# kurtkuehnert/bevy_terrain

Hardware: AMD Instinct MI355X
Metric: terrain tiles/sec preprocessed (16k^2 heightmap) (higher is better)
Workload: dtype f32; 1 GPU; synthetic 16384x16384 fBm R16 heightmap (seed 42), T=512, b=2, lod_count=6: split + pyramid + stitch into 1365 tiles; jobs_in_flight=1, ranks_seen=1, all_gather_bytes_per_rank=0

## Files before the change

### bevy_terrain_amd/csrc/bt_fused.hip

```cpp
#include <cstdio>
#include <cstdlib>
#include <type_traits>

#include "bt_internal.hpp"

namespace bt {

namespace {

constexpr uint32_t kInvalid = 0xFFFFFFFFu;

#include "bt_stitch.hpp"

#ifdef BT_DEBUG_HOOKS
#define BT_ABLATE(A, bits) ((A).ablate & (bits))
#else
#define BT_ABLATE(A, bits) 0u
#endif
constexpr uint32_t kMainRows = 8;
#ifndef BT_DMA_POS
#define BT_DMA_POS 0
#endif

constexpr uint32_t kDmaPos = BT_DMA_POS;
constexpr uint32_t kMaxBorder = 8;

struct MainItem {
    uint32_t side, x, y, atlas_index, raster;
};

struct FusedArgs {
    AttachmentMeta m;
    uint16_t* atlas;
    const RasterDev* rasters;
    const MainItem* items;
    const uint32_t* grids;
    uint32_t grid_lod_lo, grid_lod_hi, grid_sides;
    uint32_t regular, reg_first;
    const TaskDev* seam_tasks;
    uint32_t seam_count, seam_skip;
    uint32_t seam_pull;
    uint32_t tail_extras;
    float tlx, tly, brx, bry;
    uint32_t lod;
    uint32_t levels;
    uint32_t item_count;
    uint32_t groups;
    uint32_t sides;
    uint32_t lds_pitch;
    uint32_t lds_rows;
    uint32_t apron_lods;
    uint32_t rotate_priority;
    uint32_t apron_cols;
    uint32_t prev_zero;
    uint32_t apron_global;
    uint32_t single_buffer;
    uint32_t ablate;
};

__device__ __forceinline__ float unorm16_to_float(uint32_t t) {
    const float x = float(t);
    const float r = 1.0f / 65535.0f;
    const float q0 = x * r;
    const float e = __builtin_fmaf(-q0, 65535.0f, x);
    return __builtin_fmaf(e, r, q0);
}
__device__ __forceinline__ uint32_t float_to_unorm16(float e) {
    const float cl = __builtin_amdgcn_fmed3f(e, 0.0f, 1.0f);
    return uint32_t(0.5f + 65535.0f * cl);
}
__device__ __forceinline__ float mixf(float a, float b, float t) { return a * (1.0f - t) + b * t; }

struct Axis {
    int i0, i1;
    float fr;
};

__host__ __device__ __forceinline__ Axis split_axis(uint32_t r, uint32_t c, uint32_t tile, float scale, float lo, float hi, uint32_t dim) {
    const float tc = float(r) / float(c);
// ... 179 lines not shown
            out |= uint32_t(0.5f + (255.0f / 256.0f) * (sum * 0.25f)) << sh;
        }
        return out;
    }
    float value[4] = {0.0f, 0.0f, 0.0f, 0.0f}, count = 0.0f;
#pragma unroll
    for (int i = 0; i < 4; i++)
        if ((t[i] & 0x00FFFFFFu) != 0) {
#pragma unroll
            for (int k = 0; k < 4; k++) value[k] += unorm8_to_float((t[i] >> (8 * k)) & 0xFFu);
            count += 1.0f;
        }
    if (count == 0.0f) return 0;
    uint32_t out = 0;
#pragma unroll
    for (int k = 0; k < 4; k++) {
        const float e = value[k] / count;
        const float cl = e < 0.0f ? 0.0f : (e > 1.0f ? 1.0f : e);
        out |= uint32_t(floorf(0.5f + 255.0f * cl)) << (8 * k);
    }
    return out;
}

__device__ __forceinline__ uint32_t split_value_slow(const FusedArgs& A, const RasterDev& r, uint32_t tx, uint32_t rx, uint32_t ty,
                                                  uint32_t ry, uint32_t home_index) {
    const float scale = float(1u << A.lod);
    const uint32_t c = A.m.center_size, b = A.m.border_size, T = A.m.texture_size;
    const Axis ax = split_axis(rx, c, tx, scale, A.tlx, A.brx, r.width);
    const Axis ay = split_axis(ry, c, ty, scale, A.tly, A.bry, r.height);
    typedef const uint8_t __attribute__((address_space(1))) * global_bytes;
    typedef const uint16_t __attribute__((address_space(1))) * global_u16;
    const global_u16 row0 = (global_u16)((global_bytes)r.data + uint64_t(ay.i0) * r.pitch);
    const global_u16 row1 = (global_u16)((global_bytes)r.data + uint64_t(ay.i1) * r.pitch);
    const uint32_t t00 = row0[ax.i0], t10 = row0[ax.i1], t01 = row1[ax.i0], t11 = row1[ax.i1];
    if (t00 == 0 || t10 == 0 || t01 == 0 || t11 == 0) {
        if (home_index == kInvalid || A.prev_zero) return 0;
        return A.atlas[uint64_t(home_index) * T * T + uint64_t(b + ry) * T + b + rx];
    }
    const float top = mixf(unorm16_to_float(t00), unorm16_to_float(t10), ax.fr);
    const float bot = mixf(unorm16_to_float(t01), unorm16_to_float(t11), ax.fr);
    return float_to_unorm16(mixf(top, bot, ay.fr));
}

__device__ __forceinline__ uint32_t xcd_remap(uint32_t bid, uint32_t total) {
    const uint32_t q = total / 8u, r = total % 8u, xcd = bid % 8u, i = bid / 8u;
    return (xcd < r ? xcd * (q + 1u) : r * (q + 1u) + (xcd - r) * q) + i;
}

__device__ __forceinline__ int wave_min(int v) {
#pragma unroll
    for (int o = 32; o > 0; o >>= 1) v = min(v, __shfl_xor(v, o));
    return v;
// ... 1 lines not shown
__device__ __forceinline__ int wave_max(int v) {
#pragma unroll
    for (int o = 32; o > 0; o >>= 1) v = max(v, __shfl_xor(v, o));
    return v;
}

struct RowParam {
    int y0, y1;
    float fy;
    uint32_t pad;
};

constexpr uint32_t kMaxChunks = 64;
struct MainShared {
    int row_y0[kMaxChunks * kMainRows];
    float2 row_fy[kMaxChunks * kMainRows];
    int win_ymin[kMaxChunks];
    uint32_t win_slots[kMaxChunks];
    RowParam apron[2 * kMaxBorder];
    int xmin, xmax;
    uint32_t pad_[2];
};
static_assert(sizeof(MainShared) % 16 == 0, "LDS carve must stay 16-byte aligned");

struct Texel4 {
    float a0, a1, b0, b1;
    uint32_t za, zb;
};

__device__ __forceinline__ Texel4 convert4(uint32_t ta0, uint32_t ta1, uint32_t tb0, uint32_t tb1) {
    Texel4 r;
    r.a0 = unorm16_to_float(ta0);
    r.a1 = unorm16_to_float(ta1);
    r.b0 = unorm16_to_float(tb0);
    r.b1 = unorm16_to_float(tb1);
    r.za = min(ta0, ta1);
    r.zb = min(tb0, tb1);
    return r;
}

__device__ __forceinline__ void corner_pixels(const FusedArgs& A, uint32_t item_index, uint32_t tid, uint32_t threads) {
    const MainItem it = A.items[item_index];
    const RasterDev raster = A.rasters[it.raster];
    const uint32_t T = A.m.texture_size, b = A.m.border_size, c = A.m.center_size, o = b + c;
    const uint32_t self = grid_lookup(A, it.side, A.lod, int(it.x), int(it.y));
    for (uint32_t t = tid; t < 4 * b * b; t += threads) {
        const uint32_t corner = t / (b * b), i = (t % (b * b)) % b, j = (t % (b * b)) / b;
        const bool left = corner == 0 || corner == 3, top = corner < 2;
        const uint32_t px = left ? i : o + i, py = top ? j : o + j;
        const uint32_t n = grid_lookup(A, it.side, A.lod, int(it.x) + (left ? -1 : 1), int(it.y) + (top ? -1 : 1));
        uint32_t v;
        if (n != kInvalid)
            v = split_value_slow(A, raster, left ? it.x - 1 : it.x + 1, left ? c - b + i : i, top ? it.y - 1 : it.y + 1, top ? c - b + j : j, n);
        else
            v = split_value_slow(A, raster, it.x, left ? 0u : c - 1, it.y, top ? 0u : c - 1, self);
        A.atlas[uint64_t(self) * T * T + py * T + px] = uint16_t(v);
    }
}

template <bool kStaged, bool kGeneric, uint32_t kT, uint32_t kP, bool kDma = false>
__device__ __forceinline__ void fused_main_chunks(const FusedArgs& A, uint32_t item_index, uint32_t k_begin, uint32_t k_end, uint8_t* smem) {
    MainShared& S = *reinterpret_cast<MainShared*>(smem);
    uint16_t* s_buf = reinterpret_cast<uint16_t*>(smem + sizeof(MainShared));
    constexpr bool kFix = kStaged && !kGeneric;
    const bool one_buffer = kDma && kP == 0 && A.single_buffer != 0;
    const uint32_t buf_texels = one_buffer ? 0u : A.lds_rows * (kP ? kP : A.lds_pitch);

    const MainItem it = A.items[item_index];
    const RasterDev raster = A.rasters[it.raster];
    const uint32_t T = kT ? kT : A.m.texture_size, b = A.m.border_size, c = A.m.center_size, o = b + c;
    const uint32_t tid = threadIdx.x;
#ifdef BT_DEBUG_HOOKS
    auto wg_stamp = [&](uint32_t slot) {
        if (BT_ABLATE(A, 134217728u) && tid == 0 && blockIdx.x < 4096u)
            reinterpret_cast<unsigned long long*>(A.atlas + uint64_t(A.m.atlas_size - 1u) * T * T)[16384u + blockIdx.x * 4u + slot] = __builtin_amdgcn_s_memrealtime();
    };
#else
    auto wg_stamp = [&](uint32_t) {};
#endif
    wg_stamp(0);
    const float scale = float(1u << A.lod);
    const uint32_t tile_texels = T * T;
    const uint32_t chunks_per_tile = (c + kMainRows - 1) / kMainRows;

    const TileNb t5 = load_tile_nb(A, it.side, A.lod, it.x, it.y);
    const uint32_t self4 = A.levels >= 2 ? grid_lookup(A, it.side, A.lod - 1, int(it.x >> 1), int(it.y >> 1)) : kInvalid;
    const uint32_t self3 = A.levels >= 3 ? grid_lookup(A, it.side, A.lod - 2, int(it.x >> 2), int(it.y >> 2)) : kInvalid;

    for (uint32_t i = tid; i < (k_end - k_begin) * kMainRows; i += 256u) {
        const uint32_t cr = k_begin * kMainRows + i;
        if (cr < c) {
            const Axis ay = split_axis(cr, c, it.y, scale, A.tly, A.bry, raster.height);
            S.row_y0[i] = ay.i0 | (ay.i1 == ay.i0 ? int(0x80000000u) : 0);
            S.row_fy[i] = float2{ay.fr, 1.0f - ay.fr};
        }
    }
    if (tid >= 32 && tid < 32 + 2 * b) {
        const uint32_t r = tid - 32, k = r % b;
        const bool top = r < b;
        const uint32_t nrow = top ? t5.n : t5.s;
        uint32_t ty, ry;
        if (nrow != kInvalid) { ty = top ? it.y - 1 : it.y + 1; ry = top ? c - b + k : k; } else { ty = it.y; ry = top ? 0u : c - 1; }
        const Axis ay = split_axis(ry, c, ty, scale, A.tly, A.bry, raster.height);
        S.apron[r].y0 = ay.i0;
        S.apron[r].y1 = ay.i1;
        S.apron[r].fy = ay.fr;
        S.apron[r].pad = ry;
    }

    const uint32_t half_c = c / 2, half_b = b / 2;
    const bool is_centre = tid < half_c;
    const bool is_right = !is_centre && tid < half_c + half_b;
    const bool is_left = !is_centre && !is_right && tid < half_c + 2 * half_b;
    const bool is_idle = !is_centre && !is_right && !is_left;
    uint32_t px0 = 0;
    uint32_t txa = it.x, txb = it.x, rxa = 0, rxb = 0;
    if (is_centre) {
        px0 = b + 2 * tid;
        rxa = 2 * tid;
        rxb = 2 * tid + 1;
    } else if (is_right) {
        const uint32_t j = 2 * (tid - half_c);
        px0 = o + j;
        if (t5.e != kInvalid) { txa = txb = it.x + 1; rxa = j; rxb = j + 1; } else { rxa = rxb = c - 1; }
    } else if (is_left) {
        const uint32_t j = 2 * (tid - half_c - half_b);
        px0 = j;
        if (t5.w != kInvalid) { txa = txb = it.x - 1; rxa = c - b + j; rxb = c - b + j + 1; } else { rxa = rxb = 0; }
    }
    const Axis axa = split_axis(rxa, c, txa, scale, A.tlx, A.brx, raster.width);
    const Axis axb = split_axis(rxb, c, txb, scale, A.tlx, A.brx, raster.width);
    const float fxa = axa.fr, fxb = axb.fr, gxa = 1.0f - fxa, gxb = 1.0f - fxb;
    const uint32_t home_col = is_right && t5.e != kInvalid ? t5.e : (is_left && t5.w != kInvalid ? t5.w : t5.self);

    if (tid == half_c + half_b) S.xmin = min(axa.i0, axb.i0);
    if (tid == half_c + half_b - 1) S.xmax = max(axa.i1, axb.i1);
    __syncthreads();
    if (tid < k_end - k_begin) {
        const uint32_t k = k_begin + tid, n = min(kMainRows, c - k * kMainRows);
        const int* y0 = S.row_y0 + tid * kMainRows;
        const int first = y0[0] & 0x7fffffff;
        bool consecutive = n == kMainRows;
        for (uint32_t i = 0; i < n; i++) consecutive = consecutive && y0[i] == first + int(i);
        int lo = first, hi = (y0[n - 1] & 0x7fffffff) + (y0[n - 1] < 0 ? 0 : 1);
        if (!(kDma && kP == 0 && A.apron_global)) {
            if (k == 0) lo = min(lo, S.apron[0].y0);
            if (k == chunks_per_tile - 1) hi = max(hi, S.apron[2 * b - 1].y1);
        }
        S.win_ymin[tid] = lo;
        S.win_slots[tid] = uint32_t(hi - lo + 1) | (consecutive ? 0x80000000u : 0u);
    }
    __syncthreads();

    const int xa = __builtin_amdgcn_readfirstlane(S.xmin) & ~7;
    const uint32_t P = kP ? kP : A.lds_pitch;
    typedef const uint8_t __attribute__((address_space(1))) * global_bytes;
    typedef const uint16_t __attribute__((address_space(1))) * global_u16;
    typedef uint32_t u32x4 __attribute__((ext_vector_type(4)));
    typedef const u32x4 __attribute__((address_space(1))) * global_u4;
    typedef uint16_t u16x2 __attribute__((ext_vector_type(2)));
    const global_bytes data = (global_bytes)raster.data;
    const uint32_t chunks_per_row = P / 8u;
    const uint32_t row_texels = uint32_t(raster.pitch / 2u);
    const bool wide = ((reinterpret_cast<uintptr_t>(raster.data) | raster.pitch) & 15u) == 0;
    constexpr uint32_t kBatch = 4;

    auto chunk_rows = [&](uint32_t k) -> uint32_t { return min(kMainRows, c - k * kMainRows); };
    auto window = [&](uint32_t k, int& ymin, uint32_t& slots) {
        ymin = __builtin_amdgcn_readfirstlane(S.win_ymin[k - k_begin]);
        slots = uint32_t(__builtin_amdgcn_readfirstlane(S.win_slots[k - k_begin])) & 0x7fffffffu;
    };
    uint32_t src_off[kBatch], lds_off[kBatch];
#pragma unroll
    for (uint32_t i = 0; i < kBatch; i++) {
        const uint32_t ch = tid + 256u * i;
        const uint32_t slot = ch / chunks_per_row, kk = ch - slot * chunks_per_row;
        const uint32_t x = min(uint32_t(xa) + 8u * kk, row_texels - 8u);
        src_off[i] = slot * uint32_t(raster.pitch) + x * 2u;
        lds_off[i] = (slot * P + 8u * kk) * 2u;
    }
    const uint32_t safe_off = src_off[0] - (tid / chunks_per_row) * uint32_t(raster.pitch);
    auto stage_issue = [&](int ymin, uint32_t slots, u32x4 (&v)[kBatch]) {
        const global_bytes base = data + uint64_t(uint32_t(ymin)) * raster.pitch;
        const uint32_t bound = slots * P * 2u;
#pragma unroll
        for (uint32_t i = 0; i < kBatch; i++) {
            const global_u4 ptr = (global_u4)(base + (lds_off[i] < bound ? src_off[i] : safe_off));
            v[i] = BT_ABLATE(A, 32768u) ? __builtin_nontemporal_load(ptr) : *ptr;
        }
    };
    auto stage_commit = [&](uint16_t* s_src, uint32_t slots, const u32x4 (&v)[kBatch]) {
        const uint32_t bound = slots * P * 2u;
        uint8_t* s_bytes = reinterpret_cast<uint8_t*>(s_src);
#pragma unroll
        for (uint32_t i = 0; i < kBatch; i++)
            if (lds_off[i] < bound) *reinterpret_cast<u32x4*>(s_bytes + lds_off[i]) = v[i];
    };
    auto stage_narrow = [&](uint16_t* s_src, int ymin, uint32_t slots) {
        for (uint32_t i = tid; i < slots * P; i += 256u) {
            const uint32_t slot = i / P, kk = i - slot * P;
            const uint32_t x = uint32_t(xa) + kk;
            const global_u16 row = (global_u16)(data + uint64_t(ymin + int(slot)) * raster.pitch);
            s_src[i] = x < raster.width ? row[x] : uint16_t(1);
        }
    };

    typedef __attribute__((address_space(3))) uint8_t* lds_bytes;
    const uint32_t dma_lane = tid & 63u;
    const uint32_t dma_off_main = min(uint32_t(xa) * 2u + dma_lane * 16u, uint32_t(raster.pitch) - 16u);
    const uint32_t dma_off_tail = min(uint32_t(xa) * 2u + 1024u + (dma_lane & 1u) * 16u, uint32_t(raster.pitch) - 16u);
    auto dma_issue = [&](uint16_t* s_dst, int ymin, uint32_t slots) {
        static_assert(!kDma || kP == 528 || kP == 0, "the DMA variants: 1056-byte LDS rows, or a run-time pitch");
        const lds_bytes dst = (lds_bytes)reinterpret_cast<uint8_t*>(s_dst);
        for (uint32_t slot = uint32_t(__builtin_amdgcn_readfirstlane(int(tid >> 6))); slot < slots; slot += 4u) {
            const global_bytes row = data + uint64_t(uint32_t(ymin) + slot) * raster.pitch;
            if constexpr (kP == 528) {
                if (BT_ABLATE(A, 32768u))
                    __builtin_amdgcn_global_load_lds((const __attribute__((address_space(1))) void*)(row + dma_off_main),
                                                     (__attribute__((address_space(3))) void*)(dst + slot * (kP * 2u)), 16, 0, 2);
                else
                __builtin_amdgcn_global_load_lds((const __attribute__((address_space(1))) void*)(row + dma_off_main),
                                                 (__attribute__((address_space(3))) void*)(dst + slot * (kP * 2u)), 16, 0, 0);
                if (dma_lane < 2u)
                    __builtin_amdgcn_global_load_lds((const __attribute__((address_space(1))) void*)(row + dma_off_tail),
                                                     (__attribute__((address_space(3))) void*)(dst + slot * (kP * 2u) + 1024u), 16, 0, 0);
            } else {
                const uint32_t row_bytes = P * 2u;
                for (uint32_t piece = 0; piece < row_bytes; piece += 1024u)
                    if (piece + dma_lane * 16u < row_bytes)
                        __builtin_amdgcn_global_load_lds((const __attribute__((address_space(1))) void*)(row + min(uint32_t(xa) * 2u + piece + dma_lane * 16u, uint32_t(raster.pitch) - 16u)),
                                                         (__attribute__((address_space(3))) void*)(dst + slot * row_bytes + piece), 16, 0, 0);
            }
        }
    };

    uint16_t* tile5 = A.atlas + uint64_t(t5.self) * tile_texels;
    uint32_t* tile5_u32 = reinterpret_cast<uint32_t*>(tile5);
    uint16_t* tile4 = A.atlas + uint64_t(self4 == kInvalid ? 0u : self4) * tile_texels;
    uint16_t* tile3 = A.atlas + uint64_t(self3 == kInvalid ? 0u : self3) * tile_texels;
    const uint32_t cx4 = (it.x & 1u) * half_c + tid, cy4_base = (it.y & 1u) * half_c;
    const uint32_t cx3 = (it.x & 3u) * (c / 4) + (tid >> 1), cy3_base = (it.y & 3u) * (c / 4);
    const bool do4 = A.levels >= 2 && !BT_ABLATE(A, 1u), do3 = A.levels >= 3 && !BT_ABLATE(A, 1u);
    auto make_xpush = [&](uint32_t shift, uint32_t self, uint32_t cx, uint32_t& layer, uint32_t& off, uint32_t& count) {
        layer = 0;
        off = 0;
        count = 0;
        if (!is_centre || self == kInvalid) return;
        const bool left = cx < b, right = cx >= c - b;
        if (!left && !right) return;
        const uint32_t n = grid_lookup(A, it.side, A.lod - shift, int(it.x >> shift) + (left ? -1 : 1), int(it.y >> shift));
        const uint32_t j = left ? cx : cx - (c - b);
        if (n != kInvalid) {
            layer = n;
            off = b * T + (left ? o + j : j);
            count = 1;
        } else if (left ? cx == 0 : cx == c - 1) {
            layer = self;
            off = b * T + (left ? 0u : o);
            count = b;
        }
    };
    uint32_t x4_layer, x4_off, x4_count, x3_layer, x3_off, x3_count;
    make_xpush(1, A.levels >= 2 ? self4 : kInvalid, cx4, x4_layer, x4_off, x4_count);
    make_xpush(2, A.levels >= 3 ? self3 : kInvalid, cx3, x3_layer, x3_off, x3_count);
    auto xpush4 = [&](uint32_t cy, uint16_t v) {
        for (uint32_t e = 0; e < x4_count; e++) A.atlas[uint64_t(x4_layer) * tile_texels + x4_off + cy * T + e] = v;
    };
    auto xpush3 = [&](uint32_t cy, uint16_t v) {
        for (uint32_t e = 0; e < x3_count; e++) A.atlas[uint64_t(x3_layer) * tile_texels + x3_off + cy * T + e] = v;
    };
    const uint32_t la0 = uint32_t(axa.i0 - xa), la1 = uint32_t(axa.i1 - xa), lb0 = uint32_t(axb.i0 - xa), lb1 = uint32_t(axb.i1 - xa);

    int ymin = 0;
    uint32_t slots = 0;
    u32x4 pre[kBatch];
    window(k_begin, ymin, slots);
    if constexpr (kDma) {
        dma_issue(s_buf + (k_begin & 1u) * buf_texels, ymin, slots);
    } else if (kStaged && !BT_ABLATE(A, 8u)) {
        if (wide) {
            stage_issue(ymin, slots, pre);
            stage_commit(s_buf + (k_begin & 1u) * buf_texels, slots, pre);
        } else {
            stage_narrow(s_buf + (k_begin & 1u) * buf_texels, ymin, slots);
        }
    }
    if constexpr (kStaged) {
        if (k_begin == 0) corner_pixels(A, item_index, tid, 256u);
    }
    auto chunk_barrier = [&]() {
        if constexpr (kDma) asm volatile("s_waitcnt vmcnt(0)" ::: "memory");
        __syncthreads();
    };
    uint16_t* s_src = s_buf;
    int cur_ymin = 0;
    auto fetch_row = [&](int y) -> Texel4 {
        if constexpr (kStaged) {
            const uint16_t* row = s_src + uint32_t(y - cur_ymin) * P;
            return convert4(row[la0], row[la1], row[lb0], row[lb1]);
        } else {
            const global_u16 row = (global_u16)(data + uint64_t(y) * raster.pitch);
            return convert4(row[axa.i0], row[axa.i1], row[axb.i0], row[axb.i1]);
        }
    };
    auto apron_rows = [&](uint32_t k, auto gtag) {
        constexpr bool kKeep = decltype(gtag)::value;
        if (!((k == 0 || k == chunks_per_tile - 1) && is_centre)) return;
        for (uint32_t r = 0; r < 2 * b; r++) {
            const bool top = r < b;
            if (top ? k != 0 : k != chunks_per_tile - 1) continue;
            const uint32_t kk = r % b, py = top ? kk : o + kk;
            const int y0 = __builtin_amdgcn_readfirstlane(S.apron[r].y0), y1 = __builtin_amdgcn_readfirstlane(S.apron[r].y1);
// ... 371 lines not shown
                            xpush4(cy4, uint16_t(q0));
                            xpush4(cy4 + 1, uint16_t(q1));
                        }
                        if (do3) {
                            const uint32_t other0 = __shfl_xor(q0, 1), other1 = __shfl_xor(q1, 1);
                            if (is_centre && (tid & 1u) == 0) {
                                const f2 mine = conv2(q0, q1), theirs = conv2(other0, other1);
                                const float s3 = ((mine.x + mine.y) + theirs.x) + theirs.y;
                                uint32_t w3 = uint32_t(0.5f + (0.25f * (65535.0f / 65536.0f)) * s3);
                                if (kFix && min(min(q0, q1), min(other0, other1)) == 0) w3 = downsample4(q0, q1, other0, other1);
                                const uint32_t cy3 = cy3_base + (cy >> 2);
                                tile3[(b + cy3) * T + b + cx3] = uint16_t(w3);
                                if (x3_count) xpush3(cy3, uint16_t(w3));
                            }
                        }
                    }
                }
                }
            } else {
                generic_rows(k);
            }
        }

        if (!more) break;
        if (kStaged && !kDma && !BT_ABLATE(A, 8u)) {
            uint16_t* s_next = s_buf + ((k + 1) & 1u) * buf_texels;
            if (wide) stage_commit(s_next, next_slots, pre);
            else stage_narrow(s_next, next_ymin, next_slots);
        }
        ymin = next_ymin;
        slots = next_slots;
        if constexpr (kDma && kP == 0) {
            if (one_buffer) {
                __syncthreads();
                dma_issue(s_buf, next_ymin, next_slots);
            }
        }
        chunk_barrier();
    }
    wg_stamp(2);
#ifdef BT_DEBUG_HOOKS
    if (BT_ABLATE(A, 134217728u) && tid == 0)
        reinterpret_cast<unsigned long long*>(A.atlas + uint64_t(A.m.atlas_size - 1u) * tile_texels)[item_index * 8u + 4u] = __builtin_amdgcn_s_memrealtime();
#endif
    wg_stamp(3);
}

template <bool kStaged, bool kGeneric, uint32_t kT, uint32_t kP, bool kDma = false>
__global__ __launch_bounds__(256) __attribute__((amdgpu_waves_per_eu(4, 4))) void fused_main_kernel(FusedArgs A) {
    extern __shared__ __attribute__((aligned(16))) uint8_t smem[];
    const uint32_t work = BT_ABLATE(A, 1024u) ? blockIdx.x : xcd_remap(blockIdx.x, gridDim.x);
    const uint32_t chunks_per_tile = (A.m.center_size + kMainRows - 1) / kMainRows;
    const uint32_t part = work % A.groups;
    const uint32_t k_begin = part * chunks_per_tile / A.groups, k_end = (part + 1) * chunks_per_tile / A.groups;
    if (k_begin >= k_end) return;
#ifdef BT_DEBUG_HOOKS
#define BT_FUSED_DEBUG_ENTRY_PRIORITY
#include "bt_fused_debug.inc"
#undef BT_FUSED_DEBUG_ENTRY_PRIORITY
#endif
    fused_main_chunks<kStaged, kGeneric, kT, kP, kDma>(A, work / A.groups, k_begin, k_end, smem);
// ... 849 lines not shown
        if (unorm16_to_float(t) != float(t) / d) atomicAdd(failures, 1u);
        const float x = float(t);
        if (__builtin_fmaf(x, 1.0f / 65535.0f, x) != 65536.0f * (x / d)) atomicAdd(failures, 1u);
    }
    if (t < 256u) {
        volatile float d = 255.0f;
        const float x = float(t), r = 1.0f / 255.0f, q0 = x * r;
        if (__builtin_fmaf(__builtin_fmaf(-q0, 255.0f, x), r, q0) != x / d) atomicAdd(failures, 1u);
        if (__builtin_fmaf(x, r, x) != 256.0f * (x / d)) atomicAdd(failures, 1u);
    }
}

}


struct FusedJobDev {
    FusedArgs args;
    uint32_t attachment;
    uint32_t queue_job = 0;
    uint32_t lds_pad = 0;
    std::vector<MainItem> host_items;
    uint32_t seam_first = 0;
    std::vector<uint32_t> finest_layers, all_layers;
};

struct FusedState {
    std::vector<FusedJobDev> jobs;
    void* arrays = nullptr;
    std::vector<uint8_t> whole_raster;
};

}

#include <algorithm>
namespace bt {

static FusedState& state_of(bt_preprocessor* p) {
    if (!p->fused) p->fused = new FusedState();
    return *p->fused;
}

void fused_release(bt_preprocessor* p) {
    if (!p->fused) return;
    hipFree(p->fused->arrays);
    delete p->fused;
    p->fused = nullptr;
// ... 343 lines not shown
    }
    uint64_t buffers = 2;
    if (dma_variant && fixed + 2 * rows_needed * pitch * 2 > kQuarter && fixed + core_rows * pitch * 2 <= kQuarter) {
        A.single_buffer = 1;
        A.apron_global = 1;
        rows_needed = core_rows;
        buffers = 1;
    }
    const bool fits_lds = buffers * rows_needed * pitch * 2 <= budget && (rows_needed + 1) * max_pitch < (1ull << 31);
    const bool fits_batch = rows_needed * (pitch / 8) <= 256 * 4;
    const bool dma_only = fits_lds && aligned && pitch <= 4096 && (!fits_batch || m.texture_size == 512);
    A.lds_rows = fits_lds && (fits_batch || dma_only) ? uint32_t(rows_needed) : 0u;
    if ((A.apron_global || A.single_buffer) && A.lds_rows && !dma_only) {
        A.apron_global = 0;
        A.single_buffer = 0;
        A.lds_rows = 0;
    }
    if (!A.lds_rows) return BT_VARIANT_MAIN_UNSTAGED;
    if (aligned && m.texture_size == 512 && A.lds_pitch == 528) return BT_VARIANT_MAIN_DMA_528;
    if (dma_only) return A.single_buffer ? BT_VARIANT_MAIN_SINGLE_BUFFER : A.apron_global ? BT_VARIANT_MAIN_APRON_GLOBAL : BT_VARIANT_MAIN_DMA_PITCH;
    return BT_VARIANT_MAIN_REG_PITCH;
}

static void plan_main(const bt_preprocessor* p, const JobPlan& j, PlanOut& out) {
    FusedJobDev job = main_job(j);
#ifdef BT_DEBUG_HOOKS
    if (const char* e = getenv("BT_FUSED_LDS_PAD")) job.lds_pad = uint32_t(atoi(e));
#endif
    {
        const uint32_t chunks = (j.m.center_size + kMainRows - 1) / kMainRows;
        uint32_t parts = 1;
#ifdef BT_DEBUG_HOOKS
        if (const char* e = getenv("BT_FUSED_PARTS")) parts = uint32_t(atoi(e));
        else
#endif
        {
            while (parts < chunks && uint64_t(j.items.size()) * parts < 1024) parts++;
            for (uint32_t cand = parts; cand <= std::min(chunks, parts + 8); cand++)
                if ((uint64_t(j.items.size()) * cand) % 1024 == 0) { parts = cand; break; }
        }
        parts = std::max(parts, (chunks + kMaxChunks - 1) / kMaxChunks);
        job.args.groups = std::max(1u, std::min(parts, chunks));
    }
    Launch lm = job_launch(j, kLaunchFusedMain, size_main_window(p, j, job.args));
    job.args.rotate_priority = 1;
    lm.kernels = lm.variant == BT_VARIANT_MAIN_UNSTAGED ? 2u : 1u;
    lm.task_count = uint32_t(j.items.size());
    lm.aux0 = uint32_t(out.state.jobs.size());
    lm.algorithmic_bytes = main_bytes(j);
    out.state.jobs.push_back(job);
    out.plan.push_back(lm);
}

static void plan_apron_stitch(const JobPlan& j, PlanOut& out) {
    if (j.main_levels <= 1 || j.rows_in_tail()) return;
    Launch ls = job_launch(j, kLaunchStitch, BT_VARIANT_STITCH_LAUNCH);
    ls.first_task = uint32_t(out.tasks.size());
    for (const Task* t : j.stitches)
        if (t->coord.lod != j.grid.lod_hi && t->coord.lod + j.main_levels > j.grid.lod_hi) out.tasks.push_back(to_device_task(*t));
    ls.task_count = uint32_t(out.tasks.size()) - ls.first_task;
    ls.algorithmic_bytes = uint64_t(ls.task_count) * j.apron_bytes();
    ls.phase = j.shard ? 2u : 0u;
    ls.aux0 = (j.shard || j.direct) ? 0u : 1u;
    if (!j.shard && !j.direct) ls.algorithmic_bytes = uint64_t(ls.task_count) * 2 * (2 * j.m.border_size * uint64_t(j.m.texture_size)) * j.m.pixel_size;
    if (ls.task_count) out.plan.push_back(ls);
}

struct TailPlan {
// ... 90 lines not shown
                            const uint32_t pairs = (m.format != BT_FORMAT_R16 || ((m.border_size | m.texture_size) & 1u)) ? pixels : pixels / 2u;
                            parts = std::max(1u, std::min(255u, (pairs + 255u) / 256u));
                            e.rel_index[i] = (t->rel[i].coordinate.x << 16) | t->rel[i].coordinate.y;
                        }
                        for (uint32_t part = 0; part < parts; part++) {
                            if (pulled) e.raster = (main_lo - t->coord.lod) | (part << 8) | (parts << 16);
                            out.tasks.push_back(e);
                        }
                        (pass == 0 ? tail_pixels : late_pixels) += uint64_t(m.border_size) * (i < 4 ? m.center_size : m.border_size);
                    }
            }
        if (pass == 0) continue;
        Launch ls = job_launch(j, kLaunchStitch, BT_VARIANT_STITCH_LAUNCH);
        ls.aux0 = 2u;
        ls.first_task = first;
        ls.task_count = uint32_t(out.tasks.size()) - first;
        ls.algorithmic_bytes = 2 * late_pixels * m.pixel_size;
        ls.phase = j.shard ? 2u : 0u;
        if (ls.task_count) out.plan.push_back(ls);
    }
}

static bt_status fused_upload(FusedState& state, const std::vector<std::vector<MainItem>>& items, const std::vector<std::vector<uint32_t>>& grids) {
    std::vector<size_t> at(2 * items.size());
    size_t bytes = 0;
    for (size_t k = 0; k < at.size(); k++) {
        at[k] = (bytes + 255) & ~size_t(255);
        bytes = at[k] + (k % 2 ? grids[k / 2].size() * sizeof(uint32_t) : items[k / 2].size() * sizeof(MainItem));
    }
    BT_HIP(hipMalloc(&state.arrays, bytes ? bytes : 1));
    uint8_t* base = (uint8_t*)state.arrays;
    for (size_t k = 0; k < items.size(); k++) {
        if (!items[k].empty()) BT_HIP(hipMemcpy(base + at[2 * k], items[k].data(), items[k].size() * sizeof(MainItem), hipMemcpyHostToDevice));
        if (!grids[k].empty()) BT_HIP(hipMemcpy(base + at[2 * k + 1], grids[k].data(), grids[k].size() * sizeof(uint32_t), hipMemcpyHostToDevice));
    }
    for (FusedJobDev& job : state.jobs) {
        job.args.items = (const MainItem*)(base + at[2 * job.queue_job]);
        job.args.grids = (const uint32_t*)(base + at[2 * job.queue_job + 1]);
    }
    return BT_OK;
}

bool fused_plan(bt_preprocessor* p, bt_atlas* a, std::vector<TaskDev>& tasks, std::vector<Launch>& plan) {
    FusedState& state = state_of(p);
    hipFree(state.arrays);
    state.arrays = nullptr;
    state.jobs.clear();
    state.whole_raster.assign(p->rasters.size(), 0);
    if (p->queue.empty()) return false;

    PlanOut out{tasks, plan, state};
    std::vector<std::vector<MainItem>> items;
    std::vector<std::vector<uint32_t>> grids;
    for (uint32_t job = 0; job < p->jobs; job++) {
        JobPlan j;
        if (!collect_job(p, a, job, j) || !fill_grid(j) || !qualifies(j)) return false;
        plan_shards(p, j);
        order_items(p, j);
        describe_job(p, a, j);
        if (j.hybrid) plan_hybrid(j, out);
        else if (j.direct) plan_direct(p, j, out);
// ... 119 lines not shown
}

void fused_launch_tiles(const bt_preprocessor* p, const Launch& l, uint32_t item_begin, uint32_t item_count, std::vector<FusedTile>* out) {
    out->clear();
    if ((l.kind != kLaunchFusedMain && l.kind != kLaunchFusedDirect) || !p->fused || l.aux0 >= p->fused->jobs.size()) return;
    const FusedJobDev& job = p->fused->jobs[l.aux0];
    for (uint64_t i = item_begin; i < uint64_t(item_begin) + item_count && i < job.host_items.size(); i++) {
        const MainItem& it = job.host_items[size_t(i)];
        out->push_back({{it.side, job.args.lod, it.x, it.y}, it.atlas_index});
    }
}

bt_status fused_launch_range(bt_preprocessor* p, bt_atlas* a, const Launch& l, uint32_t item_begin, uint32_t item_count) {
    (void)a;
    if (!p->fused || l.aux0 >= p->fused->jobs.size()) {
        set_error("fused launch without a plan");
        return BT_ERR_INVALID_ARGUMENT;
    }
    FusedJobDev job = p->fused->jobs[l.aux0];
    FusedArgs& A = job.args;
    A.rasters = p->rasters_dev;
    if ((l.kind == kLaunchFusedMain || l.kind == kLaunchFusedDirect) && item_begin < A.item_count) {
        A.items += item_begin;
        A.item_count = std::min(item_count, A.item_count - item_begin);
    }
    const hipStream_t stream = p->ctx->stream;
    auto direct_blocks = [&] {
        const uint32_t blocks_per_tile = (A.m.center_size + kDirectRows - 1) / kDirectRows;
        return A.item_count * ((blocks_per_tile + A.groups - 1) / A.groups);
    };
    const uint32_t main_blocks = A.item_count * A.groups;
    const size_t main_lds = std::min<size_t>(65536, sizeof(MainShared) + (A.single_buffer ? 1 : 2) * size_t(A.lds_rows) * A.lds_pitch * 2 + job.lds_pad);
    switch (l.variant) {
        case BT_VARIANT_DIRECT:
            fused_direct_rgba8_kernel<false><<<direct_blocks(), 256, 0, stream>>>(A);
            break;
        case BT_VARIANT_DIRECT_REP:
            fused_direct_rgba8_kernel<true><<<direct_blocks(), 256, 0, stream>>>(A);
            break;
        case BT_VARIANT_DIRECT_SKIPS:
            fused_direct_rgba8_kernel<false, true><<<direct_blocks(), 256, 0, stream>>>(A);
            break;
        case BT_VARIANT_MAIN_DMA_528:
            fused_main_kernel<true, false, 512, 528, true><<<main_blocks, 256, main_lds, stream>>>(A);
            break;
        case BT_VARIANT_MAIN_DMA_PITCH:
// ... 63 lines not shown
```

Measured before the change: 4.663 million tiles/s.

## Precompute per-tile setup tables on host and load them in main kernel

Moves per-workgroup setup (row/column interpolation axes, neighbour grid lookups, window bounds, apron and corner axes) into a host-built blob uploaded once at plan time, deduplicated by tile row/column. The kernel now reads these records instead of running split_axis and grid_lookup and two barriers, and issues the first staging load before filling LDS tables. Corner pixels are deferred to later in the chunk loop and use precomputed axes. It also restructures narrow staging to loop per row. The risk is extra global reads of setup records and a larger plan-time upload.

```diff
diff --git a/bevy_terrain_amd/csrc/bt_fused.hip b/bevy_terrain_amd/csrc/bt_fused.hip
--- a/bevy_terrain_amd/csrc/bt_fused.hip
+++ b/bevy_terrain_amd/csrc/bt_fused.hip
@@ -1,5 +1,7 @@
 #include <cstdio>
+#include <array>
 #include <cstdlib>
+#include <cstring>
 #include <type_traits>
 
 #include "bt_internal.hpp"
@@ -28,6 +30,8 @@
 struct MainItem {
     uint32_t side, x, y, atlas_index, raster;
 };
+
+struct MainSetup;
 
 struct FusedArgs {
     AttachmentMeta m;
@@ -55,6 +59,9 @@
     uint32_t prev_zero;
     uint32_t apron_global;
     uint32_t single_buffer;
+    const MainSetup* setup;
+    const uint8_t* setup_tables;
+    uint32_t one_raster;
     uint32_t ablate;
 };
 
@@ -280,12 +287,17 @@
     return out;
 }
 
+__device__ __forceinline__ uint32_t split_value_at(const FusedArgs& A, const RasterDev& r, const Axis& ax, uint32_t rx, const Axis& ay, uint32_t ry, uint32_t home_index);
 __device__ __forceinline__ uint32_t split_value_slow(const FusedArgs& A, const RasterDev& r, uint32_t tx, uint32_t rx, uint32_t ty,
                                                   uint32_t ry, uint32_t home_index) {
     const float scale = float(1u << A.lod);
-    const uint32_t c = A.m.center_size, b = A.m.border_size, T = A.m.texture_size;
+    const uint32_t c = A.m.center_size;
     const Axis ax = split_axis(rx, c, tx, scale, A.tlx, A.brx, r.width);
     const Axis ay = split_axis(ry, c, ty, scale, A.tly, A.bry, r.height);
+    return split_value_at(A, r, ax, rx, ay, ry, home_index);
+}
+__device__ __forceinline__ uint32_t split_value_at(const FusedArgs& A, const RasterDev& r, const Axis& ax, uint32_t rx, const Axis& ay, uint32_t ry, uint32_t home_index) {
+    const uint32_t b = A.m.border_size, T = A.m.texture_size;
     typedef const uint8_t __attribute__((address_space(1))) * global_bytes;
     typedef const uint16_t __attribute__((address_space(1))) * global_u16;
     const global_u16 row0 = (global_u16)((global_bytes)r.data + uint64_t(ay.i0) * r.pitch);
@@ -333,6 +345,27 @@
     uint32_t pad_[2];
 };
 static_assert(sizeof(MainShared) % 16 == 0, "LDS carve must stay 16-byte aligned");
+
+struct MainSetup {
+    uint32_t side, x, y, raster;
+    uint32_t self, n, e, s, w;
+    uint32_t self4, self3;
+    uint32_t p4w, p4e, p3w, p3e;
+    int xmin, xmax;
+    uint32_t rows_at, cols_at;
+    uint32_t pad_;
+    RowParam apron[2 * kMaxBorder];
+    int win_ymin[kMaxChunks];
+    uint32_t win_slots[kMaxChunks];
+    uint32_t diag[4];
+    Axis corner_x[4][kMaxBorder], corner_y[4][kMaxBorder];
+};
+static_assert(sizeof(MainSetup) % 16 == 0, "records and the tables behind them stay 16-byte aligned");
+struct ColParam {
+    int a0, a1, b0, b1;
+    float fa, fb;
+    uint32_t pad_[2];
+};
 
 struct Texel4 {
     float a0, a1, b0, b1;
@@ -369,6 +402,19 @@
     }
 }
 
+__device__ __forceinline__ void corner_pixels_setup(const FusedArgs& A, const MainSetup& R, const RasterDev& raster, uint32_t tid) {
+    const uint32_t T = A.m.texture_size, b = A.m.border_size, c = A.m.center_size, o = b + c;
+    for (uint32_t t = tid; t < 4 * b * b; t += 256u) {
+        const uint32_t corner = t / (b * b), i = (t % (b * b)) % b, j = (t % (b * b)) / b;
+        const bool left = corner == 0 || corner == 3, top = corner < 2;
+        const uint32_t px = left ? i : o + i, py = top ? j : o + j;
+        const uint32_t n = R.diag[corner];
+        const uint32_t rx = n != kInvalid ? (left ? c - b + i : i) : (left ? 0u : c - 1), ry = n != kInvalid ? (top ? c - b + j : j) : (top ? 0u : c - 1);
+        const uint32_t v = split_value_at(A, raster, R.corner_x[corner][i], rx, R.corner_y[corner][j], ry, n != kInvalid ? n : R.self);
+        A.atlas[uint64_t(R.self) * T * T + py * T + px] = uint16_t(v);
+    }
+}
+
 template <bool kStaged, bool kGeneric, uint32_t kT, uint32_t kP, bool kDma = false>
 __device__ __forceinline__ void fused_main_chunks(const FusedArgs& A, uint32_t item_index, uint32_t k_begin, uint32_t k_end, uint8_t* smem) {
     MainShared& S = *reinterpret_cast<MainShared*>(smem);
@@ -377,8 +423,9 @@
     const bool one_buffer = kDma && kP == 0 && A.single_buffer != 0;
     const uint32_t buf_texels = one_buffer ? 0u : A.lds_rows * (kP ? kP : A.lds_pitch);
 
-    const MainItem it = A.items[item_index];
-    const RasterDev raster = A.rasters[it.raster];
+    const MainSetup& R = A.setup[item_index];
+    const RasterDev raster = A.rasters[A.one_raster != kInvalid ? A.one_raster : R.raster];
+    const MainItem it{R.side, R.x, R.y, R.self, R.raster};
     const uint32_t T = kT ? kT : A.m.texture_size, b = A.m.border_size, c = A.m.center_size, o = b + c;
     const uint32_t tid = threadIdx.x;
 #ifdef BT_DEBUG_HOOKS
@@ -390,80 +437,13 @@
     auto wg_stamp = [&](uint32_t) {};
 #endif
     wg_stamp(0);
-    const float scale = float(1u << A.lod);
     const uint32_t tile_texels = T * T;
     const uint32_t chunks_per_tile = (c + kMainRows - 1) / kMainRows;
 
-    const TileNb t5 = load_tile_nb(A, it.side, A.lod, it.x, it.y);
-    const uint32_t self4 = A.levels >= 2 ? grid_lookup(A, it.side, A.lod - 1, int(it.x >> 1), int(it.y >> 1)) : kInvalid;
-    const uint32_t self3 = A.levels >= 3 ? grid_lookup(A, it.side, A.lod - 2, int(it.x >> 2), int(it.y >> 2)) : kInvalid;
-
-    for (uint32_t i = tid; i < (k_end - k_begin) * kMainRows; i += 256u) {
-        const uint32_t cr = k_begin * kMainRows + i;
-        if (cr < c) {
-            const Axis ay = split_axis(cr, c, it.y, scale, A.tly, A.bry, raster.height);
-            S.row_y0[i] = ay.i0 | (ay.i1 == ay.i0 ? int(0x80000000u) : 0);
-            S.row_fy[i] = float2{ay.fr, 1.0f - ay.fr};
-        }
-    }
-    if (tid >= 32 && tid < 32 + 2 * b) {
-        const uint32_t r = tid - 32, k = r % b;
-        const bool top = r < b;
-        const uint32_t nrow = top ? t5.n : t5.s;
-        uint32_t ty, ry;
-        if (nrow != kInvalid) { ty = top ? it.y - 1 : it.y + 1; ry = top ? c - b + k : k; } else { ty = it.y; ry = top ? 0u : c - 1; }
-        const Axis ay = split_axis(ry, c, ty, scale, A.tly, A.bry, raster.height);
-        S.apron[r].y0 = ay.i0;
-        S.apron[r].y1 = ay.i1;
-        S.apron[r].fy = ay.fr;
-        S.apron[r].pad = ry;
-    }
-
-    const uint32_t half_c = c / 2, half_b = b / 2;
-    const bool is_centre = tid < half_c;
-    const bool is_right = !is_centre && tid < half_c + half_b;
-    const bool is_left = !is_centre && !is_right && tid < half_c + 2 * half_b;
-    const bool is_idle = !is_centre && !is_right && !is_left;
-    uint32_t px0 = 0;
-    uint32_t txa = it.x, txb = it.x, rxa = 0, rxb = 0;
-    if (is_centre) {
-        px0 = b + 2 * tid;
-        rxa = 2 * tid;
-        rxb = 2 * tid + 1;
-    } else if (is_right) {
-        const uint32_t j = 2 * (tid - half_c);
-        px0 = o + j;
-        if (t5.e != kInvalid) { txa = txb = it.x + 1; rxa = j; rxb = j + 1; } else { rxa = rxb = c - 1; }
-    } else if (is_left) {
-        const uint32_t j = 2 * (tid - half_c - half_b);
-        px0 = j;
-        if (t5.w != kInvalid) { txa = txb = it.x - 1; rxa = c - b + j; rxb = c - b + j + 1; } else { rxa = rxb = 0; }
-    }
-    const Axis axa = split_axis(rxa, c, txa, scale, A.tlx, A.brx, raster.width);
-    const Axis axb = split_axis(rxb, c, txb, scale, A.tlx, A.brx, raster.width);
-    const float fxa = axa.fr, fxb = axb.fr, gxa = 1.0f - fxa, gxb = 1.0f - fxb;
-    const uint32_t home_col = is_right && t5.e != kInvalid ? t5.e : (is_left && t5.w != kInvalid ? t5.w : t5.self);
-
-    if (tid == half_c + half_b) S.xmin = min(axa.i0, axb.i0);
-    if (tid == half_c + half_b - 1) S.xmax = max(axa.i1, axb.i1);
-    __syncthreads();
-    if (tid < k_end - k_begin) {
-        const uint32_t k = k_begin + tid, n = min(kMainRows, c - k * kMainRows);
-        const int* y0 = S.row_y0 + tid * kMainRows;
-        const int first = y0[0] & 0x7fffffff;
-        bool consecutive = n == kMainRows;
-        for (uint32_t i = 0; i < n; i++) consecutive = consecutive && y0[i] == first + int(i);
-        int lo = first, hi = (y0[n - 1] & 0x7fffffff) + (y0[n - 1] < 0 ? 0 : 1);
-        if (!(kDma && kP == 0 && A.apron_global)) {
-            if (k == 0) lo = min(lo, S.apron[0].y0);
-            if (k == chunks_per_tile - 1) hi = max(hi, S.apron[2 * b - 1].y1);
-        }
-        S.win_ymin[tid] = lo;
-        S.win_slots[tid] = uint32_t(hi - lo + 1) | (consecutive ? 0x80000000u : 0u);
-    }
-    __syncthreads();
-
-    const int xa = __builtin_amdgcn_readfirstlane(S.xmin) & ~7;
+    const TileNb t5{R.self, R.n, R.e, R.s, R.w};
+    const uint32_t self4 = R.self4, self3 = R.self3;
+
+    const int xa = R.xmin & ~7;
     const uint32_t P = kP ? kP : A.lds_pitch;
     typedef const uint8_t __attribute__((address_space(1))) * global_bytes;
     typedef const uint16_t __attribute__((address_space(1))) * global_u16;
@@ -508,11 +488,12 @@
             if (lds_off[i] < bound) *reinterpret_cast<u32x4*>(s_bytes + lds_off[i]) = v[i];
     };
     auto stage_narrow = [&](uint16_t* s_src, int ymin, uint32_t slots) {
-        for (uint32_t i = tid; i < slots * P; i += 256u) {
-            const uint32_t slot = i / P, kk = i - slot * P;
-            const uint32_t x = uint32_t(xa) + kk;
+        for (uint32_t slot = 0; slot < slots; slot++) {
             const global_u16 row = (global_u16)(data + uint64_t(ymin + int(slot)) * raster.pitch);
-            s_src[i] = x < raster.width ? row[x] : uint16_t(1);
+            for (uint32_t kk = tid; kk < P; kk += 256u) {
+                const uint32_t x = uint32_t(xa) + kk;
+                s_src[slot * P + kk] = x < raster.width ? row[x] : uint16_t(1);
+            }
         }
     };
 
@@ -545,6 +526,60 @@
         }
     };
 
+    int ymin = R.win_ymin[k_begin];
+    uint32_t slots = R.win_slots[k_begin] & 0x7fffffffu;
+    u32x4 pre[kBatch];
+    if constexpr (kDma) {
+        dma_issue(s_buf + (k_begin & 1u) * buf_texels, ymin, slots);
+    } else if (kStaged && !BT_ABLATE(A, 8u)) {
+        if (wide) stage_issue(ymin, slots, pre);
+    }
+    {
+        const uint32_t run_rows = (k_end - k_begin) * kMainRows;
+        const int* g_y0 = reinterpret_cast<const int*>(A.setup_tables + R.rows_at);
+        const float2* g_fy = reinterpret_cast<const float2*>(g_y0 + chunks_per_tile * kMainRows);
+        for (uint32_t i = tid; i < run_rows; i += 256u) {
+            S.row_y0[i] = g_y0[k_begin * kMainRows + i];
+            S.row_fy[i] = g_fy[k_begin * kMainRows + i];
+        }
+        if (tid < k_end - k_begin) {
+            S.win_ymin[tid] = R.win_ymin[k_begin + tid];
+            S.win_slots[tid] = R.win_slots[k_begin + tid];
+        }
+        if (tid >= 32 && tid < 32 + 2 * b) S.apron[tid - 32] = R.apron[tid - 32];
+    }
+
+    const uint32_t half_c = c / 2, half_b = b / 2;
+    const bool is_centre = tid < half_c;
+    const bool is_right = !is_centre && tid < half_c + half_b;
+    const bool is_left = !is_centre && !is_right && tid < half_c + 2 * half_b;
+    const bool is_idle = !is_centre && !is_right && !is_left;
+    uint32_t px0 = 0;
+    uint32_t rxa = 0, rxb = 0;
+    if (is_centre) {
+        px0 = b + 2 * tid;
+        rxa = 2 * tid;
+        rxb = 2 * tid + 1;
+    } else if (is_right) {
+        const uint32_t j = 2 * (tid - half_c);
+        px0 = o + j;
+        if (t5.e != kInvalid) { rxa = j; rxb = j + 1; } else { rxa = rxb = c - 1; }
+    } else if (is_left) {
+        const uint32_t j = 2 * (tid - half_c - half_b);
+        px0 = j;
+        if (t5.w != kInvalid) { rxa = c - b + j; rxb = c - b + j + 1; } else { rxa = rxb = 0; }
+    }
+    const ColParam col = reinterpret_cast<const ColParam*>(A.setup_tables + R.cols_at)[tid];
+    const Axis axa{col.a0, col.a1, col.fa}, axb{col.b0, col.b1, col.fb};
+    const float fxa = axa.fr, fxb = axb.fr, gxa = 1.0f - fxa, gxb = 1.0f - fxb;
+    const uint32_t home_col = is_right && t5.e != kInvalid ? t5.e : (is_left && t5.w != kInvalid ? t5.w : t5.self);
+    if constexpr (kStaged && !kDma) {
+        if (!BT_ABLATE(A, 8u)) {
+            if (wide) stage_commit(s_buf + (k_begin & 1u) * buf_texels, slots, pre);
+            else stage_narrow(s_buf + (k_begin & 1u) * buf_texels, ymin, slots);
+        }
+    }
+
     uint16_t* tile5 = A.atlas + uint64_t(t5.self) * tile_texels;
     uint32_t* tile5_u32 = reinterpret_cast<uint32_t*>(tile5);
     uint16_t* tile4 = A.atlas + uint64_t(self4 == kInvalid ? 0u : self4) * tile_texels;
@@ -552,14 +587,14 @@
     const uint32_t cx4 = (it.x & 1u) * half_c + tid, cy4_base = (it.y & 1u) * half_c;
     const uint32_t cx3 = (it.x & 3u) * (c / 4) + (tid >> 1), cy3_base = (it.y & 3u) * (c / 4);
     const bool do4 = A.levels >= 2 && !BT_ABLATE(A, 1u), do3 = A.levels >= 3 && !BT_ABLATE(A, 1u);
-    auto make_xpush = [&](uint32_t shift, uint32_t self, uint32_t cx, uint32_t& layer, uint32_t& off, uint32_t& count) {
+    auto make_xpush = [&](uint32_t self, uint32_t west, uint32_t east, uint32_t cx, uint32_t& layer, uint32_t& off, uint32_t& count) {
         layer = 0;
         off = 0;
         count = 0;
         if (!is_centre || self == kInvalid) return;
         const bool left = cx < b, right = cx >= c - b;
         if (!left && !right) return;
-        const uint32_t n = grid_lookup(A, it.side, A.lod - shift, int(it.x >> shift) + (left ? -1 : 1), int(it.y >> shift));
+        const uint32_t n = left ? west : east;
         const uint32_t j = left ? cx : cx - (c - b);
         if (n != kInvalid) {
             layer = n;
@@ -572,8 +607,8 @@
         }
     };
     uint32_t x4_layer, x4_off, x4_count, x3_layer, x3_off, x3_count;
-    make_xpush(1, A.levels >= 2 ? self4 : kInvalid, cx4, x4_layer, x4_off, x4_count);
-    make_xpush(2, A.levels >= 3 ? self3 : kInvalid, cx3, x3_layer, x3_off, x3_count);
+    make_xpush(A.levels >= 2 ? self4 : kInvalid, R.p4w, R.p4e, cx4, x4_layer, x4_off, x4_count);
+    make_xpush(A.levels >= 3 ? self3 : kInvalid, R.p3w, R.p3e, cx3, x3_layer, x3_off, x3_count);
     auto xpush4 = [&](uint32_t cy, uint16_t v) {
         for (uint32_t e = 0; e < x4_count; e++) A.atlas[uint64_t(x4_layer) * tile_texels + x4_off + cy * T + e] = v;
     };
@@ -582,23 +617,6 @@
     };
     const uint32_t la0 = uint32_t(axa.i0 - xa), la1 = uint32_t(axa.i1 - xa), lb0 = uint32_t(axb.i0 - xa), lb1 = uint32_t(axb.i1 - xa);
 
-    int ymin = 0;
-    uint32_t slots = 0;
-    u32x4 pre[kBatch];
-    window(k_begin, ymin, slots);
-    if constexpr (kDma) {
-        dma_issue(s_buf + (k_begin & 1u) * buf_texels, ymin, slots);
-    } else if (kStaged && !BT_ABLATE(A, 8u)) {
-        if (wide) {
-            stage_issue(ymin, slots, pre);
-            stage_commit(s_buf + (k_begin & 1u) * buf_texels, slots, pre);
-        } else {
-            stage_narrow(s_buf + (k_begin & 1u) * buf_texels, ymin, slots);
-        }
-    }
-    if constexpr (kStaged) {
-        if (k_begin == 0) corner_pixels(A, item_index, tid, 256u);
-    }
     auto chunk_barrier = [&]() {
         if constexpr (kDma) asm volatile("s_waitcnt vmcnt(0)" ::: "memory");
         __syncthreads();
@@ -1016,6 +1034,9 @@
             }
         }
 
+        if constexpr (kStaged && kDma) {
+            if (k_begin == 0 && k == (k_end - 1u) / 2u) corner_pixels_setup(A, A.setup[item_index], raster, tid);
+        }
         if (!more) break;
         if (kStaged && !kDma && !BT_ABLATE(A, 8u)) {
             uint16_t* s_next = s_buf + ((k + 1) & 1u) * buf_texels;
@@ -1031,6 +1052,9 @@
             }
         }
         chunk_barrier();
+    }
+    if constexpr (kStaged && !kDma) {
+        if (k_begin == 0) corner_pixels_setup(A, A.setup[item_index], raster, tid);
     }
     wg_stamp(2);
 #ifdef BT_DEBUG_HOOKS
@@ -1926,6 +1950,7 @@
     std::vector<MainItem> host_items;
     uint32_t seam_first = 0;
     std::vector<uint32_t> finest_layers, all_layers;
+    std::vector<uint8_t> setup;
 };
 
 struct FusedState {
@@ -2315,6 +2340,139 @@
     return BT_VARIANT_MAIN_REG_PITCH;
 }
 
+static void build_main_setup(const bt_preprocessor* p, const JobPlan& j, FusedJobDev& job, bool pitch_dma) {
+    FusedArgs& A = job.args;
+    const uint32_t c = A.m.center_size, b = A.m.border_size, lod = A.lod, n = 1u << lod;
+    const uint32_t chunks = (c + kMainRows - 1) / kMainRows, table_rows = chunks * kMainRows;
+    const uint32_t half_c = c / 2, half_b = b / 2;
+    const float scale = float(n);
+    auto lookup = [&](uint32_t side, uint32_t l, int x, int y) -> uint32_t {
+        const int nn = int(1u << l);
+        if (x < 0 || y < 0 || x >= nn || y >= nn) return kInvalid;
+        const bt_tile_coordinate at{side, l, uint32_t(x), uint32_t(y)};
+        return j.grid.holds(at) ? j.grid.cell(at) : kInvalid;
+    };
+    const std::vector<MainItem>& items = job.host_items;
+    std::vector<uint8_t>& blob = job.setup;
+    blob.assign(items.size() * sizeof(MainSetup), 0);
+    auto append = [&](size_t bytes) {
+        const size_t at = (blob.size() + 15) & ~size_t(15);
+        blob.resize(at + bytes, 0);
+        return uint32_t(at);
+    };
+    std::vector<std::pair<std::pair<uint32_t, uint32_t>, uint32_t>> row_tables;
+    std::vector<std::pair<std::array<uint32_t, 4>, uint32_t>> col_tables;
+    A.one_raster = items.empty() ? kInvalid : items[0].raster;
+    for (size_t i = 0; i < items.size(); i++) {
+        const MainItem& it = items[i];
+        if (it.raster != A.one_raster) A.one_raster = kInvalid;
+        const RasterDev& r = p->rasters[it.raster].dev;
+        const int ix = int(it.x), iy = int(it.y);
+        MainSetup R{};
+        R.side = it.side; R.x = it.x; R.y = it.y; R.raster = it.raster;
+        R.self = lookup(it.side, lod, ix, iy);
+        R.n = lookup(it.side, lod, ix, iy - 1);
+        R.e = lookup(it.side, lod, ix + 1, iy);
+        R.s = lookup(it.side, lod, ix, iy + 1);
+        R.w = lookup(it.side, lod, ix - 1, iy);
+        R.self4 = R.p4w = R.p4e = R.self3 = R.p3w = R.p3e = kInvalid;
+        if (A.levels >= 2) {
+            R.self4 = lookup(it.side, lod - 1, ix >> 1, iy >> 1);
+            R.p4w = lookup(it.side, lod - 1, (ix >> 1) - 1, iy >> 1);
+            R.p4e = lookup(it.side, lod - 1, (ix >> 1) + 1, iy >> 1);
+        }
+        if (A.levels >= 3) {
+            R.self3 = lookup(it.side, lod - 2, ix >> 2, iy >> 2);
+            R.p3w = lookup(it.side, lod - 2, (ix >> 2) - 1, iy >> 2);
+            R.p3e = lookup(it.side, lod - 2, (ix >> 2) + 1, iy >> 2);
+        }
+        {
+            const std::pair<uint32_t, uint32_t> key(it.y, it.raster);
+            auto f = std::find_if(row_tables.begin(), row_tables.end(), [&](const auto& e) { return e.first == key; });
+            if (f == row_tables.end()) {
+                const uint32_t at = append(table_rows * (sizeof(int) + sizeof(float2)));
+                std::vector<int> y0(table_rows, 0);
+                std::vector<float2> fy(table_rows, float2{0.0f, 0.0f});
+                for (uint32_t cr = 0; cr < c; cr++) {
+                    const Axis ay = split_axis(cr, c, it.y, scale, A.tly, A.bry, r.height);
+                    y0[cr] = ay.i0 | (ay.i1 == ay.i0 ? int(0x80000000u) : 0);
+                    fy[cr] = float2{ay.fr, 1.0f - ay.fr};
+                }
+                memcpy(blob.data() + at, y0.data(), table_rows * sizeof(int));
+                memcpy(blob.data() + at + table_rows * sizeof(int), fy.data(), table_rows * sizeof(float2));
+                row_tables.push_back({key, at});
+                f = row_tables.end() - 1;
+            }
+            R.rows_at = f->second;
+        }
+        {
+            const std::array<uint32_t, 4> key{it.x, it.raster, R.e != kInvalid ? 1u : 0u, R.w != kInvalid ? 1u : 0u};
+            auto f = std::find_if(col_tables.begin(), col_tables.end(), [&](const auto& e) { return e.first == key; });
+            if (f == col_tables.end()) {
+                const uint32_t at = append(256 * sizeof(ColParam));
+                std::vector<ColParam> cols(256);
+                for (uint32_t tid = 0; tid < 256; tid++) {
+                    const bool is_centre = tid < half_c, is_right = !is_centre && tid < half_c + half_b, is_left = !is_centre && !is_right && tid < half_c + 2 * half_b;
+                    uint32_t txa = it.x, txb = it.x, rxa = 0, rxb = 0;
+                    if (is_centre) {
+                        rxa = 2 * tid;
+                        rxb = 2 * tid + 1;
+                    } else if (is_right) {
+                        const uint32_t jj = 2 * (tid - half_c);
+                        if (R.e != kInvalid) { txa = txb = it.x + 1; rxa = jj; rxb = jj + 1; } else { rxa = rxb = c - 1; }
+                    } else if (is_left) {
+                        const uint32_t jj = 2 * (tid - half_c - half_b);
+                        if (R.w != kInvalid) { txa = txb = it.x - 1; rxa = c - b + jj; rxb = c - b + jj + 1; } else { rxa = rxb = 0; }
+                    }
+                    const Axis axa = split_axis(rxa, c, txa, scale, A.tlx, A.brx, r.width), axb = split_axis(rxb, c, txb, scale, A.tlx, A.brx, r.width);
+                    cols[tid] = ColParam{axa.i0, axa.i1, axb.i0, axb.i1, axa.fr, axb.fr, {0u, 0u}};
+                }
+                memcpy(blob.data() + at, cols.data(), 256 * sizeof(ColParam));
+                col_tables.push_back({key, at});
+                f = col_tables.end() - 1;
+            }
+            R.cols_at = f->second;
+            const ColParam* cols = reinterpret_cast<const ColParam*>(blob.data() + R.cols_at);
+            R.xmin = std::min(cols[half_c + half_b].a0, cols[half_c + half_b].b0);
+            R.xmax = std::max(cols[half_c + half_b - 1].a1, cols[half_c + half_b - 1].b1);
+        }
+        for (uint32_t corner = 0; corner < 4; corner++) {
+            const bool left = corner == 0 || corner == 3, top = corner < 2;
+            const uint32_t d = R.diag[corner] = lookup(it.side, lod, ix + (left ? -1 : 1), iy + (top ? -1 : 1));
+            const uint32_t tx = d == kInvalid ? it.x : (left ? it.x - 1 : it.x + 1), ty = d == kInvalid ? it.y : (top ? it.y - 1 : it.y + 1);
+            for (uint32_t q = 0; q < b; q++) {
+                const uint32_t rx = d != kInvalid ? (left ? c - b + q : q) : (left ? 0u : c - 1), ry = d != kInvalid ? (top ? c - b + q : q) : (top ? 0u : c - 1);
+                R.corner_x[corner][q] = split_axis(rx, c, tx, scale, A.tlx, A.brx, r.width);
+                R.corner_y[corner][q] = split_axis(ry, c, ty, scale, A.tly, A.bry, r.height);
+            }
+        }
+        for (uint32_t q = 0; q < 2 * b; q++) {
+            const uint32_t k = q % b;
+            const bool top = q < b;
+            uint32_t ty, ry;
+            if ((top ? R.n : R.s) != kInvalid) { ty = top ? it.y - 1 : it.y + 1; ry = top ? c - b + k : k; } else { ty = it.y; ry = top ? 0u : c - 1; }
+            const Axis ay = split_axis(ry, c, ty, scale, A.tly, A.bry, r.height);
+            R.apron[q] = RowParam{ay.i0, ay.i1, ay.fr, ry};
+        }
+        const int* table_y0 = reinterpret_cast<const int*>(blob.data() + R.rows_at);
+        for (uint32_t k = 0; k < chunks; k++) {
+            const uint32_t rows = std::min(kMainRows, c - k * kMainRows);
+            const int* y0 = table_y0 + k * kMainRows;
+            const int first = y0[0] & 0x7fffffff;
+            bool consecutive = rows == kMainRows;
+            for (uint32_t q = 0; q < rows; q++) consecutive = consecutive && y0[q] == first + int(q);
+            int lo = first, hi = (y0[rows - 1] & 0x7fffffff) + (y0[rows - 1] < 0 ? 0 : 1);
+            if (!(pitch_dma && A.apron_global)) {
+                if (k == 0) lo = std::min(lo, R.apron[0].y0);
+                if (k == chunks - 1) hi = std::max(hi, R.apron[2 * b - 1].y1);
+            }
+            R.win_ymin[k] = lo;
+            R.win_slots[k] = uint32_t(hi - lo + 1) | (consecutive ? 0x80000000u : 0u);
+        }
+        memcpy(blob.data() + i * sizeof(MainSetup), &R, sizeof(MainSetup));
+    }
+}
+
 static void plan_main(const bt_preprocessor* p, const JobPlan& j, PlanOut& out) {
     FusedJobDev job = main_job(j);
 #ifdef BT_DEBUG_HOOKS
@@ -2337,6 +2495,7 @@
     }
     Launch lm = job_launch(j, kLaunchFusedMain, size_main_window(p, j, job.args));
     job.args.rotate_priority = 1;
+    build_main_setup(p, j, job, lm.variant == BT_VARIANT_MAIN_DMA_PITCH || lm.variant == BT_VARIANT_MAIN_APRON_GLOBAL || lm.variant == BT_VARIANT_MAIN_SINGLE_BUFFER);
     lm.kernels = lm.variant == BT_VARIANT_MAIN_UNSTAGED ? 2u : 1u;
     lm.task_count = uint32_t(j.items.size());
     lm.aux0 = uint32_t(out.state.jobs.size());
@@ -2473,11 +2632,15 @@
 }
 
 static bt_status fused_upload(FusedState& state, const std::vector<std::vector<MainItem>>& items, const std::vector<std::vector<uint32_t>>& grids) {
-    std::vector<size_t> at(2 * items.size());
+    std::vector<size_t> at(2 * items.size()), setup_at(state.jobs.size());
     size_t bytes = 0;
     for (size_t k = 0; k < at.size(); k++) {
         at[k] = (bytes + 255) & ~size_t(255);
         bytes = at[k] + (k % 2 ? grids[k / 2].size() * sizeof(uint32_t) : items[k / 2].size() * sizeof(MainItem));
+    }
+    for (size_t k = 0; k < state.jobs.size(); k++) {
+        setup_at[k] = (bytes + 255) & ~size_t(255);
+        bytes = setup_at[k] + state.jobs[k].setup.size();
     }
     BT_HIP(hipMalloc(&state.arrays, bytes ? bytes : 1));
     uint8_t* base = (uint8_t*)state.arrays;
@@ -2485,9 +2648,15 @@
         if (!items[k].empty()) BT_HIP(hipMemcpy(base + at[2 * k], items[k].data(), items[k].size() * sizeof(MainItem), hipMemcpyHostToDevice));
         if (!grids[k].empty()) BT_HIP(hipMemcpy(base + at[2 * k + 1], grids[k].data(), grids[k].size() * sizeof(uint32_t), hipMemcpyHostToDevice));
     }
-    for (FusedJobDev& job : state.jobs) {
+    for (size_t k = 0; k < state.jobs.size(); k++) {
+        FusedJobDev& job = state.jobs[k];
         job.args.items = (const MainItem*)(base + at[2 * job.queue_job]);
         job.args.grids = (const uint32_t*)(base + at[2 * job.queue_job + 1]);
+        if (job.setup.empty()) continue;
+        BT_HIP(hipMemcpy(base + setup_at[k], job.setup.data(), job.setup.size(), hipMemcpyHostToDevice));
+        job.args.setup = (const MainSetup*)(base + setup_at[k]);
+        job.args.setup_tables = base + setup_at[k];
+        std::vector<uint8_t>().swap(job.setup);
     }
     return BT_OK;
 }
@@ -2653,6 +2822,7 @@
     A.rasters = p->rasters_dev;
     if ((l.kind == kLaunchFusedMain || l.kind == kLaunchFusedDirect) && item_begin < A.item_count) {
         A.items += item_begin;
+        if (A.setup) A.setup += item_begin;
         A.item_count = std::min(item_count, A.item_count - item_begin);
     }
     const hipStream_t stream = p->ctx->stream;
```

Result: faster. 4.716 million tiles/s (median of 6 runs) (+1.1%).
